# tiems90/mosaic

Hardware: AMD Instinct MI355X
Metric: PIP-join points/sec (H3 res 9) at 1/2/4/8 GPUs + achieved HBM GB/s (higher is better)
Workload: dtype f64

## Files before the change

mosaic_amd/csrc/capi.cpp:

```cpp
#include <hip/hip_runtime.h>

#include <algorithm>
#include <unordered_map>
#include <unordered_set>
#include <chrono>
#include <sched.h>
#include <array>
#include <atomic>
#include <cmath>
#include <cstdarg>
#include <cstdio>
#include <cstring>
#include <cstdlib>
#include <limits>
#include <string>
#include <map>
#include <functional>
#include <tuple>
#include <mutex>
#include <thread>
#include <vector>

#include "../../include/mosaic_arrow.h"
#include "../../include/mosaic_gpu.h"
// ... 1354 lines not shown
  if (cells.empty() || cells.size() * 5 < nonempty) return false;
  uint32_t g = 0;
  for (uint32_t d = std::min(kCellAnsSide, edge); d >= 4 && !g; d--)
    if (edge % d == 0 && cells.size() * d * d * 2 <= kCellAnsMaxBytes) g = d;
  if (g == 0) return false;
  A.g = g;
  A.sw = edge / g;
  A.ans.assign(cells.size() * g * g, mgpu::kCellAnsMixed);
  const double mu0 = 64 * (std::nextafter(1e7, INFINITY) - 1e7), w = A.sw;
  mgpu::parallel_for((int64_t)cells.size(), 4, [&](int64_t kb, int64_t ke, int) {
    for (int64_t i = kb; i < ke; i++) {
      const uint32_t k = cells[i];
      const uint64_t e = grid[D.base + k];
      const double x0 = (double)(D.a0 + (int64_t)(k % D.w)) * edge, y0 = (double)(D.b0 + (int64_t)(k / D.w)) * edge;
      const double mu = 1e-6 * w + mu0;
      for (uint32_t v = 0; v < g; v++)
        for (uint32_t u = 0; u < g; u++) {
          const int64_t m = pixel_answer(hv, e, x0 + u * w - mu, y0 + v * w - mu, x0 + (u + 1) * w + mu, y0 + (v + 1) * w + mu);
          if (m != kPixAnswerMixed && m < (int64_t)mgpu::kCellAnsMixed) A.ans[(size_t)i * g * g + v * g + u] = (uint16_t)m;
        }
    }
  });
  A.row.assign(D.h, 0);
  size_t i = 0;
  for (uint32_t r = 0; r < D.h; r++) {
    A.row[r] = (uint32_t)i;
    for (; i < cells.size() && cells[i] / D.w == r; i++) {
      uint64_t& e = grid[D.base + cells[i]];
      const uint64_t count = (e >> 32) & 0xFFFF, k = i - A.row[r];
      e = (e & ~(0xFFFFull << 32) & ~(1ull << 63)) | (count << 32) | ((k & 0x7FF) << 36) | ((k >> 11) << 63) |
          mgpu::kCellAnsFlag;
    }
  }
  return true;
}

}

namespace mgpu {
int32_t set_error(int32_t code, const char* fmt, ...) {
  char buf[512];
  va_list ap;
  va_start(ap, fmt);
  vsnprintf(buf, sizeof buf, fmt, ap);
  va_end(ap);
  g_err = buf;
  return code;
}
}

namespace {

constexpr size_t kWsCounters = 128;

struct WsLayout {
  size_t count, where, off, gsum, dirty, ties, recs, total;
};
constexpr int64_t kTieCap = 1 << 16;

WsLayout ws_layout(int64_t n_tiles, int64_t pool) {
  WsLayout L;
  size_t T = (size_t)std::max<int64_t>(n_tiles, 1);
  L.ties = align_up(kWsCounters, 256);
  L.count = align_up(L.ties + (size_t)(kTieCap + 1) * 8, 256);
  L.where = align_up(L.count + T * 4, 256);
  L.off = align_up(L.where + T * 8, 256);
  L.gsum = align_up(L.off + T * 8, 256);
  L.dirty = align_up(L.gsum + 2 * (T / 32 + 1) * 4, 256);
  L.recs = align_up(L.dirty + T * 4 * 4, 256);
  L.total = align_up(L.recs + (T * (size_t)mgpu::join_slot_records() + (size_t)std::max<int64_t>(pool, 0)) * 8, 256);
  return L;
}

int32_t ensure_ws(mgpu_ctx* ctx, int64_t n_tiles, int64_t pool = 0) {
  ctx->last.valid = false;
  ctx->last.async_pending = false;
  size_t need = ws_layout(n_tiles, pool).total;
  if (need <= ctx->ws_bytes) return MGPU_OK;
  if (ctx->ws) HIP_TRY(hipFree(ctx->ws));
  ctx->ws = nullptr;
  ctx->ws_bytes = 0;
  HIP_TRY(hipMalloc(&ctx->ws, need));
  ctx->ws_bytes = need;
  return MGPU_OK;
}

constexpr int64_t kTqInit = 1 << 12;
constexpr int64_t kTqHead = 64;
constexpr size_t kPinWords = 16 + 2 + 4 * kTqHead;

int32_t ensure_tq(mgpu_ctx* ctx, int64_t cap) {
  if (cap <= ctx->tq_cap) return MGPU_OK;
  if (ctx->tq) HIP_TRY(hipFree(ctx->tq));
  ctx->tq = nullptr;
  ctx->tq_cap = 0;
  HIP_TRY(hipMalloc(&ctx->tq, (size_t)(2 + 4 * cap) * 8));
  ctx->tq_cap = cap;
  return MGPU_OK;
}

int32_t ensure_ovr(mgpu_ctx* ctx, int64_t words) {
  if (words <= ctx->ovr_cap) return MGPU_OK;
  if (ctx->ovr) HIP_TRY(hipFree(ctx->ovr));
  ctx->ovr = nullptr;
  ctx->ovr_cap = 0;
  HIP_TRY(hipMalloc(&ctx->ovr, (size_t)words * 8));
  ctx->ovr_cap = words;
  return MGPU_OK;
}

hipError_t stream_wait(const mgpu_ctx* ctx, hipStream_t s) {
  const int64_t us = ctx->opt.spin_us;
  if (us > 0) {
    const auto t0 = std::chrono::steady_clock::now();
    const auto lim = std::chrono::microseconds(us);
    for (;;) {
// ... 1300 lines not shown
  if (chips->device != ctx->device)
    return fail(MGPU_E_INVALID_ARG, "chip table lives on device %d, context on device %d", chips->device, ctx->device);
  if (n < 0 || (n > 0 && (!x || !y))) return fail(MGPU_E_INVALID_ARG, "bad point arrays");
  if (capacity < 0 || (capacity > 0 && (!out_point || !out_poly))) return fail(MGPU_E_INVALID_ARG, "bad output arrays");
  if (int32_t st = set_device(ctx->device)) return st;
  int64_t tiles = mgpu::join_tiles(n);
  const int64_t pool = capacity;
  if (int32_t st = ensure_ws(ctx, tiles, pool)) return st;
  auto* base = (uint8_t*)ctx->ws;
  const WsLayout L = ws_layout(tiles, pool);
  const mgpu_options& o = ctx->opt;
  mgpu::JoinArgs a;
  a.x = x;
  a.y = y;
  a.n = n;
  a.n_tiles = tiles;
  a.res = res;
  a.res_match = (is == MGPU_BNG || chips->view.res < 0 || chips->view.res == res) ? 1 : 0;
  a.chips = chips->view;
  a.counters = (unsigned long long*)base;
  a.pool_used = a.counters + 5;
  a.n_dirty = (uint32_t*)(a.counters + 6);
  a.dirty = (uint32_t*)(base + L.dirty);
  a.pool_cap = pool;
  a.tile_count = (uint32_t*)(base + L.count);
  a.tile_where = (uint64_t*)(base + L.where);
  a.recs = (uint64_t*)(base + L.recs);
  a.tie_queue = ctx->tq;
  a.tie_cap = ctx->tq_cap;
  a.ovr = ctx->ovr;
  a.n_ovr = n_ovr;
  a.tie_host = (is == MGPU_H3 && tie_host) ? 1 : 0;
  a.pos_of = nullptr;
  mgpu::EmitArgs e;
  e.tile_count = a.tile_count;
  e.group_off = (uint64_t*)(base + L.off);
  a.group_sum = (uint32_t*)(base + L.gsum);
  a.group_cand = a.group_sum + (tiles / 32 + 1);
  e.tile_where = a.tile_where;
  e.recs = a.recs;
  e.point_id = point_id;
  e.id_base = id_base;
  e.capacity = capacity;
  e.out_point = out_point;
  e.out_poly = out_poly;
  a.valid = valid;
  a.valid_off = valid_off;
  a.mixed_idx = nullptr;
  a.mixed_res = nullptr;
  a.chunk_mixed = nullptr;
  a.extra = nullptr;
  a.n_extra = nullptr;
  a.poly_answers = 0;
  HIP_TRY(hipMemsetAsync(base, 0, kWsCounters, s));
  HIP_TRY(hipMemsetAsync(ctx->tq, 0, 16, s));
  const bool bng_grid = is == MGPU_BNG && chips->view.raster_mode == mgpu::kRasterNone &&
                        chips->view.probe_mode == mgpu::kProbeDense && o.bng_split;
  const bool split = (o.pipeline == MGPU_PIPELINE_AUTO || o.pipeline == MGPU_PIPELINE_SPLIT) && n > 0 &&
                     (chips->view.raster_mode != mgpu::kRasterNone || bng_grid) && a.res_match &&
                     (is == MGPU_H3 || res == chips->view.res) && chips->view.max_cell_chips <= 32;
  mgpu::SplitArgs sa{};
  if (split) {
    const int64_t nc = mgpu::split_chunks(n), C = mgpu::split_chunk();
    size_t off = 0;
    auto carve = [&](size_t bytes) {
      const size_t o_ = off;
      off = align_up(off + bytes, 256);
      return o_;
    };
    const size_t o_codes = carve((size_t)nc * C * 4), o_idx = carve((size_t)nc * C * 2), o_res = carve((size_t)nc * C * 8);
    const size_t o_pairs = carve(nc * 4), o_mixed = carve(nc * 4), o_cand = carve(nc * 4), o_off = carve(nc * 8);
    const size_t o_extra = carve((size_t)nc * (C / mgpu::join_tile_points()) * 4);
    if (off > ctx->split_bytes) {
      if (ctx->split_ws) HIP_TRY(hipFree(ctx->split_ws));
      ctx->split_ws = nullptr;
      ctx->split_bytes = 0;
      HIP_TRY(hipMalloc(&ctx->split_ws, off));
      ctx->split_bytes = off;
    }
    auto* sb = (uint8_t*)ctx->split_ws;
    sa.codes = sb + o_codes;
    sa.mixed_idx = (uint16_t*)(sb + o_idx);
    sa.chunk_pairs = (uint32_t*)(sb + o_pairs);
    sa.chunk_mixed = (uint32_t*)(sb + o_mixed);
    sa.chunk_off = (uint64_t*)(sb + o_off);
    a.extra = sa.extra = (uint32_t*)(sb + o_extra);
    a.n_extra = (uint32_t*)(a.counters + 7);
    a.group_sum = sa.chunk_pairs;
    a.group_cand = (uint32_t*)(sb + o_cand);
    a.mixed_idx = sa.mixed_idx;
    a.mixed_res = (uint64_t*)(sb + o_res);
    a.chunk_mixed = sa.chunk_mixed;
    sa.point_id = point_id;
    sa.id_base = id_base;
    sa.capacity = capacity;
    sa.out_point = out_point;
    sa.out_poly = out_poly;
    sa.j = a;
    HIP_TRY(hipMemsetAsync(a.group_cand, 0, nc * 4, s));
  }
  mgpu::BinArgs ba{};
  const bool binned = !split && plan_bins(o, chips, is, res, n, valid, a, ba);
  if (binned) {
    const int64_t nc = mgpu::split_chunks(n), C = mgpu::split_chunk();
    const int64_t K = mgpu::bin_chunks(n), G = mgpu::bin_groups(n), nb = (int64_t)ba.nbx * ba.nby;
    size_t off = 0;
    auto carve = [&](size_t bytes) {
      const size_t o_ = off;
      off = align_up(off + bytes, 256);
      return o_;
    };
    const size_t o_perm = carve((size_t)n * 4), o_rorig = carve((size_t)n * 8);
    const size_t o_bx = carve((size_t)n * 8), o_by = carve((size_t)n * 8),
                 o_pre = carve((size_t)K * nb * 4), o_res = carve((size_t)nc * C * 8), o_cnt = carve((size_t)K * nb * 4),
                 o_gs = carve((size_t)G * nb * 4), o_pairs = carve(nc * 4), o_off = carve(nc * 8),
                 o_gperm = carve(nc * 4), o_gcand = carve(nc * 4);
    const mgpu::ChipTableView& cv = chips->view;
    uint64_t grid_entries = 0;
    for (int f = 0; f < 20; f++) grid_entries = std::max<uint64_t>(grid_entries, (uint64_t)cv.dense[f].base + (uint64_t)cv.dense[f].w * cv.dense[f].h);
    const bool keyed = is == MGPU_H3 && cv.probe_mode == mgpu::kProbeDense && o.bin_keys && grid_entries < (1ull << 30);
    const size_t o_key = keyed ? carve((size_t)n * 4) : 0;
    if (off > ctx->bin_bytes) {
      if (ctx->bin_ws) HIP_TRY(hipFree(ctx->bin_ws));
      ctx->bin_ws = nullptr;
      ctx->bin_bytes = 0;
      HIP_TRY(hipMalloc(&ctx->bin_ws, off));
      ctx->bin_bytes = off;
    }
    auto* bb = (uint8_t*)ctx->bin_ws;
    ba.x = x;
    ba.y = y;
    ba.bx = (double*)(bb + o_bx);
    ba.by = (double*)(bb + o_by);
    ba.pre = (uint32_t*)(bb + o_pre);
    ba.perm = (uint32_t*)(bb + o_perm);
    ba.res = (uint64_t*)(bb + o_rorig);
    ba.cnt = (uint32_t*)(bb + o_cnt);
    ba.gsum = (uint32_t*)(bb + o_gs);
    ba.key = keyed ? (uint32_t*)(bb + o_key) : nullptr;
    mgpu::JoinArgs j = a;
    j.bin_key = ba.key;
    j.x = ba.bx;
    j.y = ba.by;
    j.mixed_idx = nullptr;
    j.chunk_mixed = nullptr;
    j.poly_answers = 1;
    j.pos_of = ba.perm;
    j.mixed_res = (uint64_t*)(bb + o_res);
    j.group_sum = (uint32_t*)(bb + o_gperm);
    j.group_cand = (uint32_t*)(bb + o_gcand);
    ba.s.j = j;
    ba.s.chunk_pairs = (uint32_t*)(bb + o_pairs);
// ... 786 lines not shown
```

mosaic_amd/csrc/kernels.h:

```cpp
#pragma once
#include <hip/hip_runtime.h>
#include <stdint.h>

#include "../../include/mosaic_gpu.h"
#include "chip_table.h"

namespace mgpu {

struct JoinArgs {
  const double* x;
  const double* y;
  int64_t n;
  int64_t n_tiles;
  int res;
  int res_match;
  ChipTableView chips;
  uint32_t* tile_count;
  uint32_t* group_sum;
  uint32_t* group_cand;
  uint64_t* tile_where;
  uint64_t* recs;
  int64_t pool_cap;
  unsigned long long* pool_used;
  uint32_t* dirty;
  uint32_t* n_dirty;
  unsigned long long* counters;
  uint64_t* tie_queue;
  int64_t tie_cap;
  const uint64_t* ovr;
  int64_t n_ovr;
  int tie_host;
  const uint32_t* pos_of;
  const uint16_t* mixed_idx;
  uint64_t* mixed_res;
  const uint32_t* chunk_mixed;
  uint32_t* extra;
  uint32_t* n_extra;

  const uint8_t* valid;
  int64_t valid_off;
  int poly_answers;
  const uint32_t* bin_key = nullptr;
  uint32_t* in_chunk_pairs = nullptr;
};

struct RedoArgs {
  const uint32_t* list;
  uint32_t* old;
  uint8_t* affected;
  uint32_t* changed;
  uint32_t* first;
};

struct SplitArgs {
  JoinArgs j;
  void* codes;
  uint32_t* chunk_pairs;
  uint32_t* chunk_mixed;
  uint16_t* mixed_idx;
  uint32_t* extra;
  uint64_t* chunk_off;
  const int64_t* point_id;
  int64_t id_base;
  int64_t capacity;
  int64_t* out_point;
  int32_t* out_poly;
  const uint32_t* redo_first = nullptr;
  const uint8_t* redo_affected = nullptr;
};
int64_t split_chunk();
int64_t split_chunk_tiles();
int64_t split_chunks(int64_t n);
hipError_t launch_split(int is, const SplitArgs& a, hipStream_t s, hipEvent_t after_classify, hipEvent_t after_mixed);
hipError_t launch_split_emit(int is, const SplitArgs& a, hipStream_t s);
hipError_t launch_split_redo(int is, const SplitArgs& sa, const RedoArgs& R, int64_t n, hipStream_t s);

struct BinArgs {
  SplitArgs s;
  const double* x;
  const double* y;
  double* bx;
  double* by;
  uint32_t* perm;
  uint64_t* res;
  uint32_t* cnt;
  uint32_t* pre;
  uint32_t* gsum;
  double x0, y0, inv_bx, inv_by;
  int32_t nbx, nby;
  int32_t xcd_runs;
  uint32_t* key;
};
int64_t bin_chunk();
int64_t bin_chunks(int64_t n);
int64_t bin_groups(int64_t n);
int32_t bin_max();
hipError_t launch_binned(int is, const BinArgs& a, hipStream_t s, hipEvent_t after_bin, hipEvent_t after_join);
hipError_t launch_bin_emit(const BinArgs& a, hipStream_t s);

struct EmitArgs {
  const uint32_t* tile_count;
  uint64_t* group_off;
  const uint64_t* tile_where;
  const uint64_t* recs;
  const int64_t* point_id;
  int64_t id_base;
  int64_t capacity;
  int64_t* out_point;
  int32_t* out_poly;
  const uint32_t* redo_first = nullptr;
  const uint8_t* redo_affected = nullptr;
};


hipError_t launch_cells(int is, int res, const double* x, const double* y, int64_t n, int64_t* out,
                        unsigned long long* counters, unsigned long long* ties, int64_t tie_cap,
                        uint64_t* tie_queue, int64_t tq_cap, hipStream_t s, const uint8_t* valid = nullptr,
                        int64_t voff = 0);
hipError_t launch_scatter_i64(const int64_t* pos, const int64_t* val, int64_t n, int64_t* out, hipStream_t s);
hipError_t launch_gather_xy(const double* x, const double* y, const int64_t* pos, int64_t n, double* xy,
                            hipStream_t s);
hipError_t launch_decode_internal(const int32_t* type_id, const int64_t* row_part, const int64_t* part_ring,
                                  const int64_t* ring_off, const double* xy, const uint8_t* valid, int64_t voff,
                                  int64_t n, double* x, double* y, unsigned long long* counters, hipStream_t s);
hipError_t launch_decode_points(int format, const uint8_t* data, const void* offsets, int off32, const uint8_t* valid,
// ... 29 lines not shown
```

mosaic_amd/csrc/kernels.hip:

```cpp
#include <hip/hip_runtime.h>
#include <stdint.h>

#define H3T_QUAL static __constant__ const
#include "h3_core.h"
#include "bng_core.h"
#include "pip_core.h"
#include "h3_ring.h"
#include "kernels.h"
#include "raster.h"

namespace mgpu {

#ifndef MGPU_BLOCK
#define MGPU_BLOCK 64
#endif
constexpr int kBlock = MGPU_BLOCK;
constexpr int kItems = 4;
constexpr int kTile = kBlock * kItems;
constexpr int kStreamBlock = 256;
static_assert(kTile <= 1024, "point-in-tile indices are 10 bits");

constexpr uint64_t kNoDst = ~0ULL;
constexpr int kScanGroup = 32;

// ... 290 lines not shown
    s_first[li] = r.first;
    if (SLOW) s_cnt[li] = (uint16_t)r.count;
    s_mask[li] = answer;
    return;
  }
  const uint32_t nj = r.count < (uint32_t)kMaskBits ? r.count : (uint32_t)kMaskBits;
  const uint32_t lowm = nj >= 32 ? 0xFFFFFFFFu : ((1u << nj) - 1);
  uint32_t border = ~r.core & lowm;
  for (uint32_t j = 16; j < nj; j++)
    if (t.chip_flags[r.first + j] & kChipCore) border &= ~(1u << j);
  uint32_t mask = lowm & ~border;
  if (border) {
    if (PT_STASH) s_cand_xy[li] = make_double2(px, py);
    const uint32_t nb = __popc(border);
    uint32_t j0 = atomicAdd(s_ncand, nb);
    for (uint32_t b = border; b; b &= b - 1) {
      const uint32_t j = __builtin_ctz(b);
      if (j0 < (uint32_t)CAND_CAP) {
        s_cand_pj[j0] = (uint16_t)(li | (j << 10));
        if (!PT_STASH && j0 < (uint32_t)STASH) s_cand_xy[j0] = make_double2(px, py);
      } else if (!SLOW) {
        any_tie = true;
      } else if (pip::chip_contains_strips(t, r.first + j, px, py)) {
        mask |= 1u << j;
      }
      j0++;
    }
  }
  s_first[li] = r.first;
  if (SLOW) s_cnt[li] = (uint16_t)(r.count > 0xFFFF ? 0xFFFF : r.count);
  s_mask[li] = mask;
}



#ifdef MGPU_STAMPS
#define MGPU_STAMP(ph)                                                              \
  do {                                                                              \
    if (threadIdx.x == 0) {                                                         \
      const uint64_t now = wall_clock64();                                          \
      if ((ph) > 0) atomicAdd(&a.counters[9 + (ph)], (unsigned long long)(now - st_t)); \
      st_t = now;                                                                   \
    }                                                                               \
  } while (0)
#else
#define MGPU_STAMP(ph) \
  do {             \
  } while (0)
#endif

constexpr int kChunk = 4096;
constexpr int kGTile = kTile;
constexpr int kChunkTiles = kChunk / kGTile;
constexpr int kGCandCap = 3 * kTile;
constexpr int kGMixCap = kTile;


template <int IS, bool SLOW, int G = 0>
__device__ __forceinline__ void join_tile(const JoinArgs& a, const uint32_t tile) {
  __shared__ uint32_t s_ncand, s_nmix;
  __shared__ uint32_t s_wave_tot[kBlock / 64];
  __shared__ uint32_t s_first[kTile];
  __shared__ __attribute__((aligned(16))) uint32_t s_mask[kTile];
  __shared__ uint16_t s_cnt[(SLOW || G == 0) ? kTile : 1];
  constexpr int kCap = G ? kGCandCap : kCandCap, kMix = G ? kGMixCap : kMixCap;
  constexpr int kStash = stash_of<G>();
  __shared__ __attribute__((aligned(16))) uint8_t s_buf[G ? kStash * 16 + kCap * 2 + kMix * 2 : kOutCap * 6];
  double2* s_cand_xy = (double2*)s_buf;
  uint16_t* s_cand_pj = (uint16_t*)(s_buf + kStash * 16);
  uint16_t* s_mix = (uint16_t*)(s_buf + kStash * 16 + kCap * 2);
  int32_t* s_out_poly = (int32_t*)s_buf;
  uint16_t* s_out_li = (uint16_t*)(s_buf + kOutCap * 4);
  __shared__ uint16_t s_gidx[G == 2 ? kTile : 1];

  const uint32_t chunk = G ? tile / kChunkTiles : 0u;
  const int64_t gbase = (int64_t)chunk * kChunk;
  const int64_t lbase = gbase + (int64_t)(tile % kChunkTiles) * kGTile;
  uint32_t gcount = 0;
  if (G) {
    const int64_t left = a.n - gbase;
    const uint32_t nm = G == 2 ? a.chunk_mixed[chunk] : (uint32_t)(left <= 0 ? 0 : (left < kChunk ? left : kChunk));
    const uint32_t t0 = (tile % kChunkTiles) * kGTile;
    if (nm <= t0) return;
    gcount = nm - t0 < (uint32_t)kGTile ? nm - t0 : (uint32_t)kGTile;
    if (G == 2)
      for (uint32_t li = threadIdx.x; li < (uint32_t)kTile; li += kBlock)
        s_gidx[li] = li < gcount ? a.mixed_idx[lbase + li] : (uint16_t)0;
  }
  uint32_t ckp[G == 1 ? 4 : 1];
  if (G == 1 && a.in_chunk_pairs) {
    const uint32_t s0 = 4u * threadIdx.x;
    if (s0 + 3 < gcount) {
      const uint4 q = *(const uint4*)(a.pos_of + lbase + s0);
      ckp[0] = q.x, ckp[1] = q.y, ckp[2] = q.z, ckp[3] = q.w;
    } else {
#pragma unroll
      for (int i = 0; i < 4; i++) ckp[i] = s0 + i < gcount ? a.pos_of[lbase + s0 + i] : 0u;
    }
  }
#define MGPU_PT(li) (G == 2 ? gbase + (int64_t)s_gidx[li] : G == 1 ? lbase + (li) : (int64_t)tile * kTile + (li))
#define MGPU_VALID(li) (G ? (uint32_t)(li) < gcount : (int64_t)tile * kTile + (li) < a.n)


#ifdef MGPU_STAMPS
  uint64_t st_t = 0;
#endif
// ... 979 lines not shown
  asm volatile("s_waitcnt lgkmcnt(0)\n\ts_barrier" ::: "memory");
#else
  __syncthreads();
#endif
}

__device__ __forceinline__ uint32_t chunk_excl_scan(uint32_t v, uint32_t* s_w, uint32_t* total) {
  const int lane = threadIdx.x & 63, wave = threadIdx.x >> 6;
  const uint32_t incl = wave_incl_scan(v);
  if (lane == 63) s_w[wave] = incl;
  lds_barrier();
  uint32_t before = 0, all = 0;
#pragma unroll
  for (int w = 0; w < kClsBlock / 64; w++) {
    before += w < wave ? s_w[w] : 0u;
    all += s_w[w];
  }
  *total = all;
  return before + incl - v;
}

constexpr int kEmitWin = 2048;
#ifndef MGPU_EMIT_SWZ
#define MGPU_EMIT_SWZ 1
#endif
__device__ __forceinline__ uint32_t emit_swz(uint32_t q) { return MGPU_EMIT_SWZ ? q ^ ((q >> 6) & 63u) : q; }
#ifndef MGPU_EMIT_NT
#define MGPU_EMIT_NT 1
#endif
#ifndef MGPU_EMIT_NT_OTHER
#define MGPU_EMIT_NT_OTHER 0
#endif
#ifndef MGPU_EMIT_WAVES
#define MGPU_EMIT_WAVES 5
#endif
constexpr int kEmitCls = 2048;
constexpr int kEmitMres = 512;
#ifndef MGPU_EMIT_MR
#define MGPU_EMIT_MR 1
#endif
template <int IS>
__global__ __launch_bounds__(kClsBlock) __attribute__((amdgpu_waves_per_eu(MGPU_EMIT_WAVES))) void split_emit_kernel(SplitArgs sa) {
  using Code = typename CodeOf<IS>::T;
  constexpr int kWords = kClsItems * (int)sizeof(Code) / 4;
  static_assert(kWords % 4 == 0 && kWords >= 4, "whole 16-byte code loads per thread (MGPU_CLS_BLOCK 256 or 512)");
  const JoinArgs& a = sa.j;
  const ChipTableView& t = a.chips;
  __shared__ uint32_t s_w[2][kClsBlock / 64];
  __shared__ uint32_t s_poly[kEmitWin];
  __shared__ uint16_t s_pt[kEmitWin];
  __shared__ int32_t s_cp[IS == MGPU_H3 ? kEmitCls : 1];
  __shared__ uint64_t s_mr[MGPU_EMIT_MR ? kEmitMres : 1];
  __shared__ int32_t s_mp[MGPU_EMIT_MR ? kEmitMres : 1];
  if (sa.redo_affected && blockIdx.x < *sa.redo_first && !sa.redo_affected[blockIdx.x]) return;
  const int64_t c0 = (int64_t)blockIdx.x * kChunk;
  const int64_t p0 = c0 + (int64_t)threadIdx.x * kClsItems;
  const Code kMixed = IS == MGPU_H3 ? (Code)kPixMixed : (Code)kCodeMixed32;
  uint32_t cw[kWords];
  if (p0 + kClsItems <= a.n) {
    const uint4* src = (const uint4*)((const Code*)sa.codes + p0);
#pragma unroll
    for (int i = 0; i < kWords / 4; i++) {
      const uint4 v = src[i];
      cw[4 * i] = v.x, cw[4 * i + 1] = v.y, cw[4 * i + 2] = v.z, cw[4 * i + 3] = v.w;
    }
  } else {
#pragma unroll
    for (int i = 0; i < kWords; i++) cw[i] = 0;
    const Code* cs = (const Code*)sa.codes;
    for (int k = 0; k < kClsItems; k++)
      if (p0 + k < a.n) {
        const uint32_t c = cs[p0 + k];
        if (sizeof(Code) == 2)
          cw[k >> 1] |= c << ((k & 1) * 16);
        else
          cw[k] = c;
      }
  }
  uint32_t ncp = 0;
  if (IS == MGPU_H3) {
    ncp = min(min(t.raster_ncls, t.raster_pc[0]), (uint32_t)kEmitCls);
    for (uint32_t i = threadIdx.x; i < ncp; i += kClsBlock) s_cp[i] = t.raster_cls_poly[i];
  }
  constexpr uint32_t kMr = MGPU_EMIT_MR ? (uint32_t)kEmitMres : 0u;
#if MGPU_EMIT_MR
  {
    const uint32_t nm = sa.chunk_mixed[blockIdx.x], nms = nm < kMr ? nm : kMr;
    for (uint32_t i = threadIdx.x; i < nms; i += kClsBlock) {
      const uint64_t v = a.mixed_res[c0 + i];
      const uint32_t m = (uint32_t)(v >> 32);
      s_mr[i] = v;
      s_mp[i] = __popc(m) == 1 ? t.chip_poly[(uint32_t)v + __builtin_ctz(m)] : 0;
    }
  }
#endif
  auto code = [&](int k) -> Code {
    return sizeof(Code) == 2 ? (Code)(cw[k >> 1] >> ((k & 1) * 16)) : (Code)cw[k];
  };
  auto pure = [&](Code c) -> uint64_t {
    if (IS == MGPU_H3) return t.raster_cls[(uint32_t)c];
    return (uint64_t)((uint32_t)c >> 8) | ((uint64_t)((uint32_t)c & 0xFFu) << 32);
  };
  auto mres = [&](uint32_t r) -> uint64_t { return r < kMr ? s_mr[r] : a.mixed_res[c0 + r]; };
  uint32_t nmix = 0;
#pragma unroll
  for (int k = 0; k < kClsItems; k++) nmix += code(k) == kMixed;
  uint32_t all_mixed;
  const uint32_t rank0 = chunk_excl_scan(nmix, s_w[0], &all_mixed);
  uint32_t npair = 0, r = rank0;
#pragma unroll
  for (int k = 0; k < kClsItems; k++) {
    const Code c = code(k);
    if (c == kMixed)
      npair += __popc((uint32_t)(mres(r++) >> 32));
    else if (c != 0) {
      if (IS == MGPU_H3)
        npair += c < t.raster_pc[0]   ? 1u
                 : c < t.raster_pc[1] ? 2u
                 : c < t.raster_pc[2] ? 3u
                 : c < t.raster_pc[3] ? 4u
                                      : (uint32_t)__popc((uint32_t)(pure(c) >> 32));
      else
        npair += (uint32_t)__popc((uint32_t)c & 0xFFu);
    }
  }
  uint32_t total;
  const uint32_t off0 = chunk_excl_scan(npair, s_w[1], &total);
  const uint64_t base = sa.chunk_off[blockIdx.x];
  for (uint32_t w0 = 0; w0 < total; w0 += kEmitWin) {
    if (off0 < w0 + kEmitWin && off0 + npair > w0) {
      uint32_t q = off0;
      r = rank0;
#pragma unroll
      for (int k = 0; k < kClsItems; k++) {
        const Code c = code(k);
        uint64_t v = 0;
        bool has_one = false;
        int32_t one = 0;
        if (c == kMixed) {
          const uint32_t rr = r++;
          if (rr < kMr && __popc((uint32_t)(s_mr[rr] >> 32)) == 1)
            has_one = true, one = s_mp[rr];
          else
            v = mres(rr);
        } else if (IS == MGPU_H3 && c != 0 && (uint32_t)c < ncp)
          has_one = true, one = s_cp[(uint32_t)c];
        else if (c != 0)
          v = pure(c);
        if (has_one) {
          if (q >= w0 && q < w0 + kEmitWin) {
            s_poly[emit_swz(q - w0)] = (uint32_t)one;
            s_pt[emit_swz(q - w0)] = (uint16_t)(threadIdx.x * kClsItems + k);
          }
          q++;
        }
        const uint32_t first = (uint32_t)v;
        for (uint32_t m = (uint32_t)(v >> 32); m; m &= m - 1, q++)
          if (q >= w0 && q < w0 + kEmitWin) {
            s_poly[emit_swz(q - w0)] = (uint32_t)t.chip_poly[first + __builtin_ctz(m)];
            s_pt[emit_swz(q - w0)] = (uint16_t)(threadIdx.x * kClsItems + k);
          }
      }
    }
    lds_barrier();
    const uint32_t cnt = total - w0 < (uint32_t)kEmitWin ? total - w0 : (uint32_t)kEmitWin;
    for (uint32_t i = threadIdx.x; i < cnt; i += kClsBlock) {
      const uint64_t q = base + w0 + i;
      if ((int64_t)q >= sa.capacity) break;
      const int64_t p = c0 + s_pt[emit_swz(i)];
#if MGPU_EMIT_NT
      __builtin_nontemporal_store(sa.point_id ? sa.point_id[p] : sa.id_base + p, &sa.out_point[q]);
      __builtin_nontemporal_store((int32_t)s_poly[emit_swz(i)], &sa.out_poly[q]);
#else
      sa.out_point[q] = sa.point_id ? sa.point_id[p] : sa.id_base + p;
      sa.out_poly[q] = (int32_t)s_poly[emit_swz(i)];
#endif
    }
    lds_barrier();
  }
}

// ... 1066 lines not shown

__global__ __launch_bounds__(256) void chunk_unpair_kernel(JoinArgs a, RedoArgs R) {
  __shared__ uint32_t s_w[4];
  const uint32_t chunk = R.list[blockIdx.x];
  const uint32_t nm = a.chunk_mixed[chunk];
  uint32_t mine = 0;
  for (uint32_t i = threadIdx.x; i < nm; i += 256) mine += __popc((uint32_t)(a.mixed_res[(int64_t)chunk * kChunk + i] >> 32));
  mine = wave_sum_u32(mine);
  if ((threadIdx.x & 63) == 0) s_w[threadIdx.x >> 6] = mine;
  __syncthreads();
  if (threadIdx.x == 0) {
    const uint32_t tot = s_w[0] + s_w[1] + s_w[2] + s_w[3];
    R.old[blockIdx.x] = a.group_sum[chunk];
    a.group_sum[chunk] -= tot;
    a.group_cand[chunk] = 0;
    R.affected[chunk] = 1;
    const uint32_t nt = (nm + kGTile - 1) / kGTile;
    const uint32_t q = atomicAdd(a.n_dirty, nt);
    for (uint32_t t = 0; t < nt; t++) a.dirty[q + t] = chunk * kChunkTiles + t;
  }
}

__global__ __launch_bounds__(256) void redo_compare_kernel(const uint32_t* counts, RedoArgs R, int64_t n) {
  const int64_t i = (int64_t)blockIdx.x * 256 + threadIdx.x;
  if (i < n && counts[R.list[i]] != R.old[i]) {
    atomicOr(R.changed, 1u);
    atomicMin(R.first, R.list[i]);
  }
}

hipError_t launch_join_redo(int is, const JoinArgs& a, const EmitArgs& e, const RedoArgs& R, int64_t n, hipStream_t s) {
  if (n <= 0) return hipSuccess;
  const unsigned g = (unsigned)((n + 255) / 256);
  hipLaunchKernelGGL(tile_unpair_kernel, dim3(g), dim3(256), 0, s, a, R, n);
  const unsigned fix_blocks = (unsigned)(n < kFixGrid ? n : kFixGrid);
  if (is == MGPU_H3)
    hipLaunchKernelGGL(pip_fix_kernel<MGPU_H3>, dim3(fix_blocks), dim3(kBlock), 0, s, a);
  else
    hipLaunchKernelGGL(pip_fix_kernel<MGPU_BNG>, dim3(fix_blocks), dim3(kBlock), 0, s, a);
  hipLaunchKernelGGL(redo_compare_kernel, dim3(g), dim3(256), 0, s, (const uint32_t*)a.tile_count, R, n);
  hipLaunchKernelGGL(tile_scan_kernel, dim3(1), dim3(kScanBlock), 0, s, a.group_sum, a.group_cand,
                     (a.n_tiles + kScanGroup - 1) / kScanGroup, e.group_off, a.counters, (const uint32_t*)R.changed);
  EmitArgs er = e;
  er.redo_first = R.first;
  er.redo_affected = R.affected;
  hipLaunchKernelGGL(pair_emit_kernel, dim3((unsigned)((a.n_tiles + kEmitTiles - 1) / kEmitTiles)),
                     dim3(kEmitBlock), 0, s, er, a.n_tiles);
  return hipGetLastError();
}

int64_t split_chunk() { return kChunk; }
int64_t split_chunk_tiles() { return kChunkTiles; }
int64_t split_chunks(int64_t n) { return (n + kChunk - 1) / kChunk; }

static int resident_blocks(const void* kernel, int block, size_t lds) {
  int dev = 0, cus = 0, per = 0;
  hipGetDevice(&dev);
  hipDeviceGetAttribute(&cus, hipDeviceAttributeMultiprocessorCount, dev);
  if (hipOccupancyMaxActiveBlocksPerMultiprocessor(&per, kernel, block, lds) != hipSuccess || per < 1) per = 1;
  return std::max(cus, 1) * per;
}

template <int IS>
static void launch_emit(const SplitArgs& a, int64_t nc, hipStream_t s) {
  hipLaunchKernelGGL(split_emit_kernel<IS>, dim3((unsigned)nc), dim3(kClsBlock), 0, s, a);
}

template <int IS>
static void launch_split_t(const SplitArgs& a, hipStream_t s, hipEvent_t after_classify, hipEvent_t after_mixed) {
  const int64_t nc = split_chunks(a.j.n);
  const ChipTableView& ct = a.j.chips;
  const size_t nblk = (IS == MGPU_H3 && ct.raster_blk) ? (size_t)ct.raster_bnx * ct.raster_bny : 0;
  const size_t lds = IS == MGPU_H3 ? ((nblk + 1) & ~(size_t)1) * 2 + (size_t)ct.raster_nband * 4 : 0;
  const int64_t wg = (nc + kCfyBlock / 64 - 1) / (kCfyBlock / 64);
  if (lds > 64 * 1024) {
    hipFuncSetAttribute((const void*)classify_pair_kernel<IS>, hipFuncAttributeMaxDynamicSharedMemorySize, (int)lds);
    hipFuncSetAttribute((const void*)classify_wave_kernel<IS>, hipFuncAttributeMaxDynamicSharedMemorySize, (int)lds);
  }
  if (MGPU_CFY_PAIR && ((((uintptr_t)a.j.x) | ((uintptr_t)a.j.y)) & 15) == 0) {
    const int64_t grid = std::min<int64_t>(wg, (int64_t)resident_blocks((const void*)classify_pair_kernel<IS>, kCfyBlock, lds));
    hipLaunchKernelGGL(classify_pair_kernel<IS>, dim3((unsigned)grid), dim3(kCfyBlock), lds, s, a, nc);
  } else {
    const int64_t grid = std::min<int64_t>(wg, (int64_t)resident_blocks((const void*)classify_wave_kernel<IS>, kCfyBlock, lds));
    hipLaunchKernelGGL(classify_wave_kernel<IS>, dim3((unsigned)grid), dim3(kCfyBlock), lds, s, a, nc);
  }
  if (after_classify) hipEventRecord(after_classify, s);
  hipLaunchKernelGGL(pip_mixed_kernel<IS>, dim3((unsigned)nc), dim3(kBlock), 0, s, a.j);
  const int64_t more = std::min<int64_t>(nc, (int64_t)resident_blocks((const void*)pip_mixed_more_kernel<IS>, kBlock, 0));
  hipLaunchKernelGGL(pip_mixed_more_kernel<IS>, dim3((unsigned)more), dim3(kBlock), 0, s, a.j);
  const int64_t fix = nc * kChunkTiles < kFixGrid ? nc * kChunkTiles : kFixGrid;
  hipLaunchKernelGGL((pip_mixed_fix_kernel<IS, 2>), dim3((unsigned)fix), dim3(kBlock), 0, s, a.j);
  if (after_mixed) hipEventRecord(after_mixed, s);
  hipLaunchKernelGGL(tile_scan_kernel, dim3(1), dim3(kScanBlock), 0, s, a.chunk_pairs, a.j.group_cand, nc,
                     a.chunk_off, a.j.counters);
  launch_emit<IS>(a, nc, s);
}

hipError_t launch_split(int is, const SplitArgs& a, hipStream_t s, hipEvent_t after_classify, hipEvent_t after_mixed) {
  if (a.j.n <= 0) return hipSuccess;
  if (is == MGPU_H3)
    launch_split_t<MGPU_H3>(a, s, after_classify, after_mixed);
  else
    launch_split_t<MGPU_BNG>(a, s, after_classify, after_mixed);
  return hipGetLastError();
}

hipError_t launch_split_redo(int is, const SplitArgs& sa, const RedoArgs& R, int64_t n, hipStream_t s) {
  if (n <= 0) return hipSuccess;
  const int64_t nc = split_chunks(sa.j.n);
  hipLaunchKernelGGL(chunk_unpair_kernel, dim3((unsigned)n), dim3(256), 0, s, sa.j, R);
  const int64_t most = n * kChunkTiles;
  const unsigned fix = (unsigned)(most < kFixGrid ? most : kFixGrid);
  if (is == MGPU_H3)
    hipLaunchKernelGGL((pip_mixed_fix_kernel<MGPU_H3, 2>), dim3(fix), dim3(kBlock), 0, s, sa.j);
  else
    hipLaunchKernelGGL((pip_mixed_fix_kernel<MGPU_BNG, 2>), dim3(fix), dim3(kBlock), 0, s, sa.j);
  hipLaunchKernelGGL(redo_compare_kernel, dim3((unsigned)((n + 255) / 256)), dim3(256), 0, s,
                     (const uint32_t*)sa.chunk_pairs, R, n);
  hipLaunchKernelGGL(tile_scan_kernel, dim3(1), dim3(kScanBlock), 0, s, sa.chunk_pairs, sa.j.group_cand, nc,
                     sa.chunk_off, sa.j.counters, (const uint32_t*)R.changed);
  SplitArgs sr = sa;
  sr.redo_first = R.first;
  sr.redo_affected = R.affected;
  if (is == MGPU_H3)
    launch_emit<MGPU_H3>(sr, nc, s);
  else
    launch_emit<MGPU_BNG>(sr, nc, s);
  return hipGetLastError();
}

hipError_t launch_split_emit(int is, const SplitArgs& a, hipStream_t s) {
  if (a.j.n <= 0) return hipSuccess;
  const int64_t nc = split_chunks(a.j.n);
  if (is == MGPU_H3)
    launch_emit<MGPU_H3>(a, nc, s);
  else
    launch_emit<MGPU_BNG>(a, nc, s);
  return hipGetLastError();
}

int64_t bin_chunk() { return kBinChunk; }
int64_t bin_chunks(int64_t n) { return (n + kBinChunk - 1) / kBinChunk; }
int64_t bin_groups(int64_t n) { return (bin_chunks(n) + kBinGroup - 1) / kBinGroup; }
int32_t bin_max() { return kBinMax; }

static void launch_bin_output(const BinArgs& a, hipStream_t s) {
  const int64_t n = a.s.j.n, K = bin_chunks(n), nc = split_chunks(n);
  if (!MGPU_BIN_JOIN_COUNTS)
    hipLaunchKernelGGL(bin_gather_kernel, dim3((unsigned)K), dim3(kBinBlock), 0, s, a);
  hipLaunchKernelGGL(tile_scan_kernel, dim3(1), dim3(kScanBlock), 0, s, a.s.chunk_pairs, a.s.j.group_cand, nc,
                     a.s.chunk_off, a.s.j.counters);
  if (MGPU_BIN_JOIN_COUNTS)
    hipLaunchKernelGGL(bin_emit_gather_kernel, dim3((unsigned)K), dim3(kBinBlock), 0, s, a);
  else
    hipLaunchKernelGGL(bin_emit_kernel, dim3((unsigned)nc), dim3(kClsBlock), 0, s, a);
}

template <int IS>
static void launch_binned_t(const BinArgs& a, hipStream_t s, hipEvent_t after_bin, hipEvent_t after_join) {
  const int64_t n = a.s.j.n, K = bin_chunks(n), G = bin_groups(n), nb = (int64_t)a.nbx * a.nby;
  hipLaunchKernelGGL(bin_hist_kernel, dim3((unsigned)K), dim3(kBinBlock), 0, s, a);
  hipLaunchKernelGGL(bin_colscan_kernel, dim3((unsigned)((nb + 255) / 256), (unsigned)G), dim3(256), 0, s, a, K);
  hipLaunchKernelGGL(bin_base_kernel, dim3(1), dim3(kBaseBlock), 0, s, a, G);
  if (IS == MGPU_H3 && a.key) {
    hipLaunchKernelGGL(bin_scatter_kernel<true>, dim3((unsigned)K), dim3(kBinBlock), 0, s, a);
  } else {
    hipLaunchKernelGGL(bin_scatter_kernel<false>, dim3((unsigned)K), dim3(kBinBlock), 0, s, a);
  }
  const int64_t nc = split_chunks(n), tiles = nc * kChunkTiles;
  JoinArgs j = a.s.j;
  if (MGPU_BIN_JOIN_COUNTS) {
    hipMemsetAsync(a.s.chunk_pairs, 0, (size_t)nc * sizeof(uint32_t), s);
    j.in_chunk_pairs = a.s.chunk_pairs;
// ... 47 lines not shown
```

Measured before the change: 98.40 billion.

## Replace single-block tile scan with grouped sums and per-chunk prefix in emit

Drops the single-workgroup tile_scan_kernel that serialised the chunk-offset prefix scan. A new one-wave-per-group kernel reduces chunk pair and candidate counts into 64-chunk group sums. Each emit block then computes its own base offset from the preceding group sums plus the preceding chunks in its group, and block 0 writes the totals to the counters. Group buffers move into the counter workspace so a single memset clears both, at the cost of extra redundant reads per emit block and a possible change to the redo path's use of R.changed.

```diff
diff --git a/mosaic_amd/csrc/capi.cpp b/mosaic_amd/csrc/capi.cpp
--- a/mosaic_amd/csrc/capi.cpp
+++ b/mosaic_amd/csrc/capi.cpp
@@ -1430,6 +1430,7 @@
 namespace {
 
 constexpr size_t kWsCounters = 128;
+constexpr size_t split_zero_bytes(int64_t chunks, int64_t groups) { return (size_t)groups * 16 + (size_t)chunks * 4; }
 
 struct WsLayout {
   size_t count, where, off, gsum, dirty, ties, recs, total;
@@ -1439,7 +1440,8 @@
 WsLayout ws_layout(int64_t n_tiles, int64_t pool) {
   WsLayout L;
   size_t T = (size_t)std::max<int64_t>(n_tiles, 1);
-  L.ties = align_up(kWsCounters, 256);
+  const int64_t pts = (int64_t)T * mgpu::join_tile_points();
+  L.ties = align_up(kWsCounters + split_zero_bytes(mgpu::split_chunks(pts), mgpu::split_groups(pts)), 256);
   L.count = align_up(L.ties + (size_t)(kTieCap + 1) * 8, 256);
   L.where = align_up(L.count + T * 4, 256);
   L.off = align_up(L.where + T * 8, 256);
@@ -2846,7 +2848,6 @@
   a.extra = nullptr;
   a.n_extra = nullptr;
   a.poly_answers = 0;
-  HIP_TRY(hipMemsetAsync(base, 0, kWsCounters, s));
   HIP_TRY(hipMemsetAsync(ctx->tq, 0, 16, s));
   const bool bng_grid = is == MGPU_BNG && chips->view.raster_mode == mgpu::kRasterNone &&
                         chips->view.probe_mode == mgpu::kProbeDense && o.bng_split;
@@ -2854,8 +2855,9 @@
                      (chips->view.raster_mode != mgpu::kRasterNone || bng_grid) && a.res_match &&
                      (is == MGPU_H3 || res == chips->view.res) && chips->view.max_cell_chips <= 32;
   mgpu::SplitArgs sa{};
+  if (!split) HIP_TRY(hipMemsetAsync(base, 0, kWsCounters, s));
   if (split) {
-    const int64_t nc = mgpu::split_chunks(n), C = mgpu::split_chunk();
+    const int64_t nc = mgpu::split_chunks(n), ng = mgpu::split_groups(n), C = mgpu::split_chunk();
     size_t off = 0;
     auto carve = [&](size_t bytes) {
       const size_t o_ = off;
@@ -2863,7 +2865,7 @@
       return o_;
     };
     const size_t o_codes = carve((size_t)nc * C * 4), o_idx = carve((size_t)nc * C * 2), o_res = carve((size_t)nc * C * 8);
-    const size_t o_pairs = carve(nc * 4), o_mixed = carve(nc * 4), o_cand = carve(nc * 4), o_off = carve(nc * 8);
+    const size_t o_pairs = carve(nc * 4), o_mixed = carve(nc * 4);
     const size_t o_extra = carve((size_t)nc * (C / mgpu::join_tile_points()) * 4);
     if (off > ctx->split_bytes) {
       if (ctx->split_ws) HIP_TRY(hipFree(ctx->split_ws));
@@ -2877,11 +2879,13 @@
     sa.mixed_idx = (uint16_t*)(sb + o_idx);
     sa.chunk_pairs = (uint32_t*)(sb + o_pairs);
     sa.chunk_mixed = (uint32_t*)(sb + o_mixed);
-    sa.chunk_off = (uint64_t*)(sb + o_off);
+    sa.chunk_off = nullptr;
     a.extra = sa.extra = (uint32_t*)(sb + o_extra);
     a.n_extra = (uint32_t*)(a.counters + 7);
     a.group_sum = sa.chunk_pairs;
-    a.group_cand = (uint32_t*)(sb + o_cand);
+    a.group_pairs = (unsigned long long*)(base + kWsCounters);
+    a.group_cands = a.group_pairs + ng;
+    a.group_cand = (uint32_t*)(a.group_cands + ng);
     a.mixed_idx = sa.mixed_idx;
     a.mixed_res = (uint64_t*)(sb + o_res);
     a.chunk_mixed = sa.chunk_mixed;
@@ -2891,7 +2895,7 @@
     sa.out_point = out_point;
     sa.out_poly = out_poly;
     sa.j = a;
-    HIP_TRY(hipMemsetAsync(a.group_cand, 0, nc * 4, s));
+    HIP_TRY(hipMemsetAsync(base, 0, kWsCounters + split_zero_bytes(nc, ng), s));
   }
   mgpu::BinArgs ba{};
   const bool binned = !split && plan_bins(o, chips, is, res, n, valid, a, ba);
diff --git a/mosaic_amd/csrc/kernels.h b/mosaic_amd/csrc/kernels.h
--- a/mosaic_amd/csrc/kernels.h
+++ b/mosaic_amd/csrc/kernels.h
@@ -36,6 +36,8 @@
   const uint32_t* chunk_mixed;
   uint32_t* extra;
   uint32_t* n_extra;
+  unsigned long long* group_pairs = nullptr;
+  unsigned long long* group_cands = nullptr;
 
   const uint8_t* valid;
   int64_t valid_off;
@@ -71,6 +73,7 @@
 int64_t split_chunk();
 int64_t split_chunk_tiles();
 int64_t split_chunks(int64_t n);
+int64_t split_groups(int64_t n);
 hipError_t launch_split(int is, const SplitArgs& a, hipStream_t s, hipEvent_t after_classify, hipEvent_t after_mixed);
 hipError_t launch_split_emit(int is, const SplitArgs& a, hipStream_t s);
 hipError_t launch_split_redo(int is, const SplitArgs& sa, const RedoArgs& R, int64_t n, hipStream_t s);
diff --git a/mosaic_amd/csrc/kernels.hip b/mosaic_amd/csrc/kernels.hip
--- a/mosaic_amd/csrc/kernels.hip
+++ b/mosaic_amd/csrc/kernels.hip
@@ -366,6 +366,7 @@
 constexpr int kChunk = 4096;
 constexpr int kGTile = kTile;
 constexpr int kChunkTiles = kChunk / kGTile;
+constexpr int kOffGroup = 64;
 constexpr int kGCandCap = 3 * kTile;
 constexpr int kGMixCap = kTile;
 
@@ -1451,7 +1452,20 @@
   __shared__ int32_t s_cp[IS == MGPU_H3 ? kEmitCls : 1];
   __shared__ uint64_t s_mr[MGPU_EMIT_MR ? kEmitMres : 1];
   __shared__ int32_t s_mp[MGPU_EMIT_MR ? kEmitMres : 1];
+  __shared__ unsigned long long s_pre[kClsBlock / 64];
+  if (blockIdx.x == 0 && threadIdx.x < 64) {
+    const int64_t ng = (gridDim.x + kOffGroup - 1) / kOffGroup;
+    unsigned long long tp = 0, tc = 0;
+    for (int64_t i = threadIdx.x; i < ng; i += 64) tp += a.group_pairs[i], tc += a.group_cands[i];
+    tp = wave_sum_u64(tp), tc = wave_sum_u64(tc);
+    if (threadIdx.x == 0) a.counters[0] = tp, a.counters[3] = tc;
+  }
   if (sa.redo_affected && blockIdx.x < *sa.redo_first && !sa.redo_affected[blockIdx.x]) return;
+  const uint32_t grp = blockIdx.x / kOffGroup;
+  const uint32_t pred = (blockIdx.x - blockIdx.x % kOffGroup) + threadIdx.x;
+  const unsigned long long pre_g0 = a.group_pairs[min(threadIdx.x, grp)];
+  const unsigned long long pre_g1 = a.group_pairs[min(threadIdx.x + kClsBlock, grp)];
+  const uint32_t pre_c = sa.chunk_pairs[min(pred, blockIdx.x)];
   const int64_t c0 = (int64_t)blockIdx.x * kChunk;
   const int64_t p0 = c0 + (int64_t)threadIdx.x * kClsItems;
   const Code kMixed = IS == MGPU_H3 ? (Code)kPixMixed : (Code)kCodeMixed32;
@@ -1523,9 +1537,18 @@
         npair += (uint32_t)__popc((uint32_t)c & 0xFFu);
     }
   }
+  {
+    unsigned long long pre = (threadIdx.x < grp ? pre_g0 : 0ull) + (threadIdx.x + kClsBlock < grp ? pre_g1 : 0ull) +
+                             (pred < blockIdx.x ? pre_c : 0u);
+    for (uint32_t i = threadIdx.x + 2 * kClsBlock; i < grp; i += kClsBlock) pre += a.group_pairs[i];
+    pre = wave_sum_u64(pre);
+    if ((threadIdx.x & 63) == 0) s_pre[threadIdx.x >> 6] = pre;
+  }
   uint32_t total;
   const uint32_t off0 = chunk_excl_scan(npair, s_w[1], &total);
-  const uint64_t base = sa.chunk_off[blockIdx.x];
+  uint64_t base = 0;
+#pragma unroll
+  for (int w = 0; w < kClsBlock / 64; w++) base += s_pre[w];
   for (uint32_t w0 = 0; w0 < total; w0 += kEmitWin) {
     if (off0 < w0 + kEmitWin && off0 + npair > w0) {
       uint32_t q = off0;
@@ -2698,6 +2721,7 @@
 int64_t split_chunk() { return kChunk; }
 int64_t split_chunk_tiles() { return kChunkTiles; }
 int64_t split_chunks(int64_t n) { return (n + kChunk - 1) / kChunk; }
+int64_t split_groups(int64_t n) { return (split_chunks(n) + kOffGroup - 1) / kOffGroup; }
 
 static int resident_blocks(const void* kernel, int block, size_t lds) {
   int dev = 0, cus = 0, per = 0;
@@ -2705,6 +2729,18 @@
   hipDeviceGetAttribute(&cus, hipDeviceAttributeMultiprocessorCount, dev);
   if (hipOccupancyMaxActiveBlocksPerMultiprocessor(&per, kernel, block, lds) != hipSuccess || per < 1) per = 1;
   return std::max(cus, 1) * per;
+}
+
+__global__ __launch_bounds__(kOffGroup) void group_sum_kernel(JoinArgs a, int64_t n_chunks) {
+  const int64_t c = (int64_t)blockIdx.x * kOffGroup + threadIdx.x;
+  unsigned long long p = c < n_chunks ? a.group_sum[c] : 0u, k = c < n_chunks ? a.group_cand[c] : 0u;
+  p = wave_sum_u64(p), k = wave_sum_u64(k);
+  if (threadIdx.x == 0) a.group_pairs[blockIdx.x] = p, a.group_cands[blockIdx.x] = k;
+}
+static_assert(kOffGroup == 64, "group_sum_kernel: one wave per group");
+
+static void launch_group_sums(const SplitArgs& a, int64_t nc, hipStream_t s) {
+  hipLaunchKernelGGL(group_sum_kernel, dim3((unsigned)((nc + kOffGroup - 1) / kOffGroup)), dim3(kOffGroup), 0, s, a.j, nc);
 }
 
 template <int IS>
@@ -2737,8 +2773,7 @@
   const int64_t fix = nc * kChunkTiles < kFixGrid ? nc * kChunkTiles : kFixGrid;
   hipLaunchKernelGGL((pip_mixed_fix_kernel<IS, 2>), dim3((unsigned)fix), dim3(kBlock), 0, s, a.j);
   if (after_mixed) hipEventRecord(after_mixed, s);
-  hipLaunchKernelGGL(tile_scan_kernel, dim3(1), dim3(kScanBlock), 0, s, a.chunk_pairs, a.j.group_cand, nc,
-                     a.chunk_off, a.j.counters);
+  launch_group_sums(a, nc, s);
   launch_emit<IS>(a, nc, s);
 }
 
@@ -2763,8 +2798,7 @@
     hipLaunchKernelGGL((pip_mixed_fix_kernel<MGPU_BNG, 2>), dim3(fix), dim3(kBlock), 0, s, sa.j);
   hipLaunchKernelGGL(redo_compare_kernel, dim3((unsigned)((n + 255) / 256)), dim3(256), 0, s,
                      (const uint32_t*)sa.chunk_pairs, R, n);
-  hipLaunchKernelGGL(tile_scan_kernel, dim3(1), dim3(kScanBlock), 0, s, sa.chunk_pairs, sa.j.group_cand, nc,
-                     sa.chunk_off, sa.j.counters, (const uint32_t*)R.changed);
+  launch_group_sums(sa, nc, s);
   SplitArgs sr = sa;
   sr.redo_first = R.first;
   sr.redo_affected = R.affected;
```

Result: faster. 99.88 billion, median of 6 (+1.5%).
